# vanilladucky/sde_sampler_lrds

Hardware: AMD Instinct MI355X
Metric: particle-steps/sec (batch*n_steps/wall) + log-Z abs-err vs ref (higher is better)
Workload: dtype f32

## Files before the change

sde_sampler_lrds_amd/csrc/prep_kernels.hip:

```cpp
#include "sim_device.hpp"
#include "prep_kernels.hpp"

__global__ void __launch_bounds__(256) k_weight_scales(PackArgs a) {
  __shared__ float red[256];
  float* sc = a.out + sd_off_scales(a.NT);
  {
    const int l = blockIdx.x;
    const float* W = l == 0 ? a.w_in : (l == 1 ? a.w_h1 : (l == 2 ? a.w_h2 : a.w_out));
    const int n = (l == 0 || l == 3) ? SD_H * a.d : SD_H * SD_H;
    float m = 0.0f;
    for (int i = threadIdx.x; i < n; i += 256) {
      const float v = __builtin_fabsf(W[i]);
      m = (v <= 3.0e38f) ? fmaxf(m, v) : m;
    }
    red[threadIdx.x] = m;
    __syncthreads();
    for (int s = 128; s > 0; s >>= 1) {
      if (threadIdx.x < s) red[threadIdx.x] = fmaxf(red[threadIdx.x], red[threadIdx.x + s]);
      __syncthreads();
    }
    if (threadIdx.x == 0) {
      const float mx = red[0];
      int e = 0;
      if (mx > 0.0f && (mx < 9.765625e-4f || mx >= 16384.0f)) {
// ... 58 lines not shown
      a.out[sd_off_bias(NT) + b] = v;
    }
  }
}

__device__ inline float gelu_exact(float v) { return (v * 0.5f) * (1.0f + erff(v * 0.70710678118654752440f)); }

__global__ void __launch_bounds__(64) k_time_embed(TimeEmbedArgs a) {
  __shared__ float e[128];
  __shared__ float hbuf[2][64];
  const int k = blockIdx.x, j = threadIdx.x;
  const float t = a.t_direct ? a.t_value : a.coef[static_cast<size_t>(k) * SDENG_NCOEF + a.col];
  const float arg = (a.te.coeff[j] * t) + a.te.phase[j];
  e[j] = sinf(arg);
  e[64 + j] = cosf(arg);
  __syncthreads();
  const float* in = e;
  int n_in = 128, cur = 0;
  for (int l = 0; l < a.te.n_hidden; ++l) {
    const float* W = a.te.w[l] + static_cast<size_t>(j) * n_in;
    float acc = 0.0f;
    for (int i = 0; i < n_in; ++i) acc = __builtin_fmaf(W[i], in[i], acc);
    acc += a.te.b[l][j];
    hbuf[cur][j] = gelu_exact(acc);
    __syncthreads();
    in = hbuf[cur];
    n_in = 64;
    cur ^= 1;
  }
  if (j < a.te.dim_out) {
    const float* W = a.te.w_out + static_cast<size_t>(j) * 64;
    float acc = 0.0f;
    for (int i = 0; i < 64; ++i) acc = __builtin_fmaf(W[i], in[i], acc);
    acc += a.te.b_out[j];
    if (a.clip > 0.0f) acc = clampf(acc, a.clip);
    a.out[static_cast<size_t>(k) * a.te.dim_out + j] = acc;
  }
}

__global__ void __launch_bounds__(128) k_same_var(const float* vars, int K, int d, float* same_var) {
  int differ = 0;
  for (int i = threadIdx.x; i < K * d; i += 128) differ |= vars[i] != vars[i % d];
  differ = __syncthreads_or(differ);
  if (threadIdx.x == 0) same_var[0] = differ ? 0.0f : 1.0f;
}

__global__ void __launch_bounds__(128) k_ref_tables(RefTabArgs a) {
  __shared__ float red[128];
  const int k = blockIdx.x / a.K, c = blockIdx.x % a.K;
  const float S = a.coef[static_cast<size_t>(k) * SDENG_NCOEF + 9];
  const float VA = a.coef[static_cast<size_t>(k) * SDENG_NCOEF + 10];
  const float S2 = a.coef[static_cast<size_t>(k) * SDENG_NCOEF + 11];
  const bool centred = a.centred && a.K == SD_KREG && a.same_var[0] != 0.0f;
  float* tm = a.tab + (static_cast<size_t>(k) * a.K + c) * 2 * a.dpad;
  float* tv = tm + a.dpad;
  float ls = 0.0f, quad = 0.0f;
  for (int f = threadIdx.x; f < a.dpad; f += 128) {
    float mean = 0.0f, iv = 0.0f, cen = 0.0f;
    if (f < a.d) {
      mean = S * a.means[static_cast<size_t>(c) * a.d + f];
      const float var = VA + S2 * a.vars[static_cast<size_t>(c) * a.d + f];
      iv = 1.0f / var;
      ls += logf(var);
      if (centred) {
        float sum = 0.0f;
        for (int j = 0; j < SD_KREG; ++j) sum += a.means[static_cast<size_t>(j) * a.d + f];
        cen = S * (sum * (1.0f / SD_KREG));
      }
    }
    if (centred) {
      const float dm = mean - cen;
      quad = __builtin_fmaf(dm * dm, iv, quad);
      tm[f] = dm * iv;
      tv[f] = c == 0 ? iv : (c == 1 ? cen : 0.0f);
    } else {
      tm[f] = mean;
      tv[f] = iv;
    }
  }
  red[threadIdx.x] = ls;
  __syncthreads();
  for (int s = 64; s > 0; s >>= 1) {
    if (threadIdx.x < s) red[threadIdx.x] += red[threadIdx.x + s];
    __syncthreads();
  }
  const float ls_sum = red[0];
  __syncthreads();
  red[threadIdx.x] = quad;
  __syncthreads();
  for (int s = 64; s > 0; s >>= 1) {
    if (threadIdx.x < s) red[threadIdx.x] += red[threadIdx.x + s];
    __syncthreads();
  }
  if (threadIdx.x == 0) {
    float wsum = 0.0f;
    for (int i = 0; i < a.K; ++i) wsum += a.weights ? a.weights[i] : 1.0f;
    const float w = (a.weights ? a.weights[c] : 1.0f) / wsum;
    float* cs = a.consts + (static_cast<size_t>(k) * a.K + c) * 2;
    cs[0] = 0.5f * ls_sum;
    cs[1] = centred ? logf(w) - 0.5f * red[0] : logf(w);
  }
}

__global__ void __launch_bounds__(256) k_ref_full_tables(RefFullArgs a) {
  __shared__ float invd[128];
  __shared__ float red[256];
  const int k = blockIdx.x / a.K, c = blockIdx.x % a.K;
  const float S = a.coef ? a.coef[static_cast<size_t>(k) * SDENG_NCOEF + 9] : 1.0f;
  const float VA = a.coef ? a.coef[static_cast<size_t>(k) * SDENG_NCOEF + 10] : 0.0f;
  const float S2 = a.coef ? a.coef[static_cast<size_t>(k) * SDENG_NCOEF + 11] : 1.0f;
  const int KB = sd_kb(a.NT);
  const int img_floats = a.NT * KB * 512;
  float ls = 0.0f;
  for (int j = threadIdx.x; j < 128; j += 256) {
    float iv = 0.0f;
    if (j < a.d) {
      const float var = VA + S2 * a.eigvals[static_cast<size_t>(c) * a.d + j];
      iv = 1.0f / var;
      ls += logf(var);
    }
    invd[j] = iv;
  }
  red[threadIdx.x] = ls;
  __syncthreads();
  for (int s = 128; s > 0; s >>= 1) {
    if (threadIdx.x < s) red[threadIdx.x] += red[threadIdx.x + s];
    __syncthreads();
// ... 799 lines not shown
```

sde_sampler_lrds_amd/csrc/prep_kernels.hpp:

```cpp
#pragma once
#include "sim_common.hpp"
#include "../../include/sdeng.h"

#define SD_LOGZ_MAX_BLOCKS 1024

struct PackArgs {
  int NT, d;
  const float *w_in, *b_in, *w_h1, *b_h1, *w_h2, *b_h2, *w_out, *b_out;
  float* out;
  int transpose;
  const float* scales;
};

struct TimeEmbedArgs {
  sdeng_time_embed te;
  const float* coef;
  int col;
  int t_direct;
  float t_value;
  float clip;
  float* out;
};

struct RefTabArgs {
  int K, d, dpad;
  const float* coef;
  const float *means, *vars, *weights;
  float* tab;
  float* consts;
  float* same_var;
  int centred;
};

struct RefFullArgs {
  int K, d, dpad, NT;
  const float* coef;
  const float *means, *eigvals, *eigvecs, *weights;
  float* images;
  float* means_out;
  float* consts;
};

struct RefMMArgs {
  int K, d, dpad, NT, kt;
  const float* coef;
  const float *means, *vars, *weights;
  float* images;
  float* centre;
  float* consts;
  float* same_var;
};

struct DistTabArgs {
  int K, d, dpad;
  const float *loc, *scale, *weights;
  float* tab;
  float* consts;
};

struct DistEvalArgs {
  DistDev ds;
  int B, d, dpad;
  const float* x;
  float* logp_out;
  float* score_out;
};

struct MovesArgs {
  DistEvalArgs prior, target;
  int B, d, K, keep_from, ula;
  float target_acc;
  const float* t;
  float *x, *lp, *grad, *step;
  const float *z, *u;
  unsigned seed_lo, seed_hi;
  long long chain0;
  float* samples;
  float* acc_sum;
  float* acc_last;
};
int sd_launch_moves(const MovesArgs& a, hipStream_t s);

struct TerminalArgs {
  DistDev ref, target;
// ... 18 lines not shown
```

sde_sampler_lrds_amd/csrc/sdeng_api.hip:

```cpp
#include <hip/hip_runtime.h>

#include <algorithm>
#include <cmath>
#include <cstdarg>
#include <cstdio>
#include <cstring>
#include <cstdlib>

#include "../../include/sdeng.h"
#include "prep_kernels.hpp"
#include "sim_kernel.hpp"
#include "cmcd_kernel.hpp"
#include "grad_kernel.hpp"
#include "cmcd_adjoint_kernel.hpp"
#include "metric_kernels.hpp"

int sd_launch_logreg_images(const float* X, const float* y, int n, int dw, int NT, float* image, float* y_pad, hipStream_t s);
int sd_launch_pack_square(const float* P, const float* loc, int d, int NT, float* out, float* loc_pad, hipStream_t s);

static thread_local char g_err[512] = "";
static int fail(int code, const char* fmt, ...) {
  va_list ap;
  va_start(ap, fmt);
  vsnprintf(g_err, sizeof(g_err), fmt, ap);
// ... 500 lines not shown
  SD_TRY(launch_timed(d, p.k, &c, s));
  if (eubo) return terminal(d, dpad, prior, prior, true, false, d->x_out, d->rnd_out, s);
  return terminal(d, dpad, target, target, false, true, d->x_out, d->rnd_out, s);
}

static int run_euler(const SimPlan& p, const sdeng_desc* d, float* ws, SimArgs& a, hipStream_t s) {
  SD_TRY(build_dist(d->target, d->d, 16 * p.DT, ws + p.L.target, a.target, s));
  a.clip_score = d->net.clip_score;
  return launch_timed(d, p.k, &a, s);
}

static int prepare_ref(const SimPlan& p, const sdeng_desc* d, float* ws, SimArgs& a, hipStream_t s) {
  const Layout& L = p.L;
  const int DT = p.DT, dpad = 16 * DT, K = ref_components(d), rf = p.rf;
  if (rf == RF_NONE) return 0;
  a.ref_k = K;
  a.ref_tab = ws + L.ref_tab; a.ref_consts = ws + L.ref_consts;
  a.ref_c1 = half_d_log_2pi(d->d);
  if (rf == RF_GMM_FULL) {
    if (d->N > 0) {
      RefFullArgs r;
      r.K = K; r.d = d->d; r.dpad = dpad; r.NT = DT; r.coef = p.in_slot ? nullptr : d->coef;
      r.means = d->ref.means_init; r.eigvals = d->ref.vars_init; r.eigvecs = d->ref.eigvecs; r.weights = d->ref.weights;
      r.images = ws + L.ref_tab; r.means_out = ws + L.ref_mean; r.consts = ws + L.ref_consts;
      SD_HIP(sd_launch_ref_full_tables(r, d->N, s));
    }
    a.ref_mean = ws + L.ref_mean;
    const int piece = (DT > 4 ? DT / 2 : DT) * sd_kb(DT) * 512;
    a.ref_share = (piece / 256 + SD_WAVES - 1) / SD_WAVES;
    return 0;
  }
  if (rf == RF_GMM_MM) {
    const int kt = (K + 15) / 16;
    if (d->N > 0) {
      RefMMArgs r;
      r.K = K; r.d = d->d; r.dpad = dpad; r.NT = DT; r.kt = kt; r.coef = d->coef;
      r.means = d->ref.means_init; r.vars = d->ref.vars_init; r.weights = d->ref.weights;
      r.images = ws + L.ref_tab; r.centre = ws + L.ref_mean; r.consts = ws + L.ref_consts;
      r.same_var = ws + L.ref_consts + static_cast<size_t>(d->N) * 64;
      SD_HIP(sd_launch_ref_mm_tables(r, d->N, s));
    }
    a.ref_kc = kt;
    a.ref_mean = ws + L.ref_mean;
    a.ref_share = (mm_piece(K, DT) / 256 + SD_WAVES - 1) / SD_WAVES;
    return 0;
  }
  if (d->N > 0) {
    RefTabArgs r;
    r.K = K; r.d = d->d; r.dpad = dpad; r.coef = d->coef;
    r.means = d->ref.means_init; r.vars = d->ref.vars_init; r.weights = rf != RF_GAUSS ? d->ref.weights : nullptr;
    r.tab = ws + L.ref_tab; r.consts = ws + L.ref_consts;
    r.same_var = ws + L.ref_consts + static_cast<size_t>(d->N) * K * 2;
    r.centred = (rf == RF_GMM && p.k.fam != SD_FAM_SPLIT) ? 1 : 0;
    SD_HIP(sd_launch_ref_tables(r, d->N, s));
  }
  a.ref_same_var = ws + L.ref_consts + static_cast<size_t>(d->N) * K * 2;
  if (rf == RF_GMM_BIG) {
    static const bool allow = [] { const char* e = getenv("SDENG_REF_SHARE"); return !(e && e[0] == '0'); }();
    const int cap = std::min(share_room(DT), sd_share_buf_floats(SD_SHARE_MAX)) / 256 * 256;
    const int kc_max = cap / (2 * dpad);
    if (allow && kc_max >= 1) {
      const int nch = (K + kc_max - 1) / kc_max;
      const int kc = (K + nch - 1) / nch;
      const int chunks = (kc * 2 * dpad + 255) / 256;
      a.ref_share = (chunks + SD_WAVES - 1) / SD_WAVES;
      a.ref_kc = kc;
    }
  }
  return 0;
}

static int run_sim(const SimPlan& p, const sdeng_desc* d, float* ws, SimArgs& a, hipStream_t s) {
  const Layout& L = p.L;
  const int DT = p.DT, dpad = 16 * DT;
  SD_TRY(prepare_net(d, L, ws, DT, a, s, d->N, false, 0.0f));
  SD_TRY(prepare_ref(p, d, ws, a, s));
  DistDev target, ref_dist, prior;
  SD_TRY(build_dist(d->target, d->d, dpad, ws + L.target, target, s));
  SD_TRY(build_dist(d->ref_dist, d->d, dpad, ws + L.ref_dist, ref_dist, s));
  SD_TRY(build_dist(d->prior, d->d, dpad, ws + L.prior, prior, s));
  a.target = target;
  a.prior = prior;
  const bool eubo = d->form == SDENG_FORM_EUBO;
  const bool tr = d->flags & SDENG_FLAG_TERM_REF, tt = d->flags & SDENG_FLAG_TERM_TARGET;
  if ((d->flags & SDENG_FLAG_INIT_LOGP) && !eubo) {
    SD_TRY(dist_eval(prior, d->B, d->d, dpad, d->x_in, ws + L.rnd_init, nullptr, s));
    a.rnd_init = ws + L.rnd_init;
  }
  if (eubo && (tr || tt)) {
    SD_HIP(hipMemsetAsync(ws + L.rnd_init, 0, sizeof(float) * d->B, s));
    SD_TRY(terminal(d, dpad, ref_dist, target, tr, tt, d->x_in, ws + L.rnd_init, s));
    a.rnd_init = ws + L.rnd_init;
  }
  if (p.sc == SC_LOGREG) {
    float* unused;
    SD_TRY(prepare_logreg(d, L, ws, DT, a, s, &unused));
  }
  SD_TRY(launch_timed(d, p.k, &a, s));
  if (!eubo && (tr || tt)) SD_TRY(terminal(d, dpad, ref_dist, target, tr, tt, d->x_out, d->rnd_out, s));
  if (eubo && (d->flags & SDENG_FLAG_INIT_LOGP)) SD_TRY(terminal(d, dpad, prior, prior, true, false, d->x_out, d->rnd_out, s));
  return 0;
}

extern "C" int sdeng_simulate(const sdeng_desc* desc, void* stream) {
  hipStream_t s = static_cast<hipStream_t>(stream);
  SimPlan p;
// ... 145 lines not shown
}
static int check_adjoint(const sdeng_desc* d, bool ext_score) {
  if (!d) return fail(SDENG_E_INVALID, "null descriptor");
  SD_TRY(check_abi(d));
  if (d->d < 1 || d->d > 128 || d->N < 1 || d->B < 1 || !d->coef) return fail(SDENG_E_INVALID, "bad sizes (1 <= d <= 128, N, B >= 1) or null coef");
  if (d->form != SDENG_FORM_LIN && d->form != SDENG_FORM_EM) return fail(SDENG_E_UNSUPPORTED, "kl_adjoint: forward forms LIN / EM (form %d)", d->form);
  if (d->net.ctrl_kind != SDENG_CTRL_CLIPPED &&
      !(score_like(d->net.ctrl_kind) && (ext_score || d->target.kind == SDENG_DIST_GMM_DIAG || d->target.kind == SDENG_DIST_PHI4)))
    return fail(SDENG_E_UNSUPPORTED, "kl_adjoint: ClippedCtrl, or Score / Lerp / CancelDrift control on a diagonal mixture / phi^4 target (ctrl_kind %d, "
                                     "target kind %d)", d->net.ctrl_kind, d->target.kind);
  SD_TRY(check_lerp_prior(d));
  if (d->target.kind == SDENG_DIST_CHECKERBOARD || d->prior.kind == SDENG_DIST_CHECKERBOARD)
    return fail(SDENG_E_UNSUPPORTED, "kl_adjoint: no adjoint for a checkerboard target (KL training takes the per-step path)");
  if (d->ref.kind != SDENG_REF_NONE && d->ref.kind != SDENG_REF_GAUSS_DIAG && d->ref.kind != SDENG_REF_GMM_DIAG)
    return fail(SDENG_E_UNSUPPORTED, "kl_adjoint: no reference, or a diagonal Gaussian / mixture reference (ref.kind %d)", d->ref.kind);
  if (d->ref.kind != SDENG_REF_NONE && ((d->ref.kind == SDENG_REF_GMM_DIAG && d->ref.k < 1) || !d->ref.means_init || !d->ref.vars_init))
    return fail(SDENG_E_INVALID, "reference: null means/vars or k < 1");
  if (static_cast<long long>(d->N) * d->B * d->d >= (1ll << 31)) return fail(SDENG_E_UNSUPPORTED, "N * B * d >= 2^31");
  return check_net(d->net);
}
extern "C" size_t sdeng_kl_adjoint_workspace_bytes(const sdeng_desc* d) {
  if (!d || d->d < 1 || d->d > 128 || d->N < 1) return 0;
  return adjoint_layout(d, tiles_exact(d->d)).total * sizeof(float);
}
extern "C" int sdeng_kl_adjoint(const sdeng_desc* d, const sdeng_adjoint* adj, void* stream) {
  hipStream_t s = static_cast<hipStream_t>(stream);
  SD_TRY(check_adjoint(d, adj && adj->score));
  if (!adj || !adj->xs || !adj->w || !adj->lam_in || !adj->a0 || !adj->a1 || !adj->a2 || !adj->d0 || !adj->d1 || !adj->d2 || !adj->dout)
    return fail(SDENG_E_INVALID, "kl_adjoint: null states / weights / lambda_N / per-row outputs");
  const bool ito = d->flags & SDENG_FLAG_ITO;
  if (ito && !adj->noise) return fail(SDENG_E_INVALID, "kl_adjoint: FLAG_ITO needs the normals of the trajectory");
  const bool score = d->net.ctrl_kind != SDENG_CTRL_CLIPPED;
  if (score && !adj->dst) return fail(SDENG_E_INVALID, "kl_adjoint: a score control needs the dst output");
  if (score && !adj->score) SD_TRY(check_dist(d->target, d->d));
  const int has_score = !score ? ADJ_NONE : adj->score ? ADJ_EXT : (d->target.kind == SDENG_DIST_PHI4 ? ADJ_PHI4 : ADJ_GMM);
  const int DT = tiles_exact(d->d), dpad = 16 * DT;
  KernelKey k;
  SD_TRY(select_kernel(k, SD_FAM_ADJ, DT, has_score));
  const AdjLayout A = adjoint_layout(d, DT);
  const size_t need = A.total * sizeof(float);
  if (!d->workspace || d->workspace_bytes < need) return fail(SDENG_E_WORKSPACE, "workspace %zu bytes, need %zu", d->workspace_bytes, need);
  float* ws = static_cast<float*>(d->workspace);
  AdjArgs a;
  memset(&a, 0, sizeof(a));
  SD_TRY(pack_net(d, DT, ws, ws + A.v.wt, s));
  SD_TRY(embed_times(d, d->N, false, 0.0f, ws + A.v.temb, ws + A.stheta, &a.stheta, s));
  if (d->ref.kind != SDENG_REF_NONE) {
    const int K = ref_components(d);
    RefTabArgs r;
    r.K = K; r.d = d->d; r.dpad = dpad; r.coef = d->coef;
    r.means = d->ref.means_init; r.vars = d->ref.vars_init; r.weights = d->ref.kind == SDENG_REF_GMM_DIAG ? d->ref.weights : nullptr;
    r.tab = ws + A.tab; r.consts = ws + A.consts;
    r.same_var = ws + A.consts + static_cast<size_t>(d->N) * K * 2;
    r.centred = 0;
    SD_HIP(sd_launch_ref_tables(r, d->N, s));
    a.ref_tab = ws + A.tab; a.ref_consts = ws + A.consts; a.ref_k = K;
    a.ref_c1 = half_d_log_2pi(d->d);
  }
  a.has_score = has_score;
  if (score) {
    a.score_ext = adj->score;
    if (!adj->score) SD_TRY(build_dist(d->target, d->d, dpad, ws + A.target, a.target, s));
    a.scale_score = d->net.scale_score; a.clip_score = d->net.clip_score;
    a.ctrl_kind = d->net.ctrl_kind;
    a.prior_loc = d->prior.p0; a.prior_scale = d->net.ctrl_kind == SDENG_CTRL_LERP ? d->prior.p1 : 1.0f;
    a.score_detached = adj->detach_score ? 1 : 0;
    a.dst = adj->dst;
  }
  VjpArgs& v = a.v;
  v.M = d->N * d->B; v.B = d->B; v.d = d->d; v.N = d->N;
  v.x = adj->xs; v.cot = nullptr; v.wpack = ws; v.wpack_t = ws + A.v.wt; v.temb = ws + A.v.temb;
  v.clip_model = d->net.clip_model;
  v.a0 = adj->a0; v.a1 = adj->a1; v.a2 = adj->a2; v.d0 = adj->d0; v.d1 = adj->d1; v.d2 = adj->d2; v.dout = adj->dout;
  v.trash = ws + A.v.trash;
  a.coef = d->coef; a.noise = ito ? adj->noise : nullptr; a.w = adj->w; a.lam_in = adj->lam_in; a.lam_out = adj->lam_out;
  a.lin = d->form == SDENG_FORM_LIN ? 1 : 0;
  a.ntiles_b = (d->B + 15) / 16;
  SD_HIP(k.fn(&a, s));
  return 0;
}

struct CmcdAdjLayout {
  VjpLayout v;
  size_t stheta, target, prior, total;
};
static CmcdAdjLayout cmcd_adjoint_layout(const sdeng_desc* d, int DT) {
  CmcdAdjLayout A;
  A.v = vjp_layout(DT, d->N + 1);
  size_t o = A.v.total;
  A.stheta = o; o += align64(static_cast<size_t>(d->N) + 1);
  A.target = o; o += dist_floats(d->target, 16 * DT);
  A.prior = o; o += dist_floats(d->prior, 16 * DT);
  A.total = o;
  return A;
}
static int check_cmcd_adjoint(const sdeng_desc* d, bool ext_score) {
  if (!d) return fail(SDENG_E_INVALID, "null descriptor");
  SD_TRY(check_abi(d));
  if (d->d > 128) return fail(SDENG_E_UNSUPPORTED, "cmcd_kl_adjoint: d <= 128 (got %d)", d->d);
  if (d->d < 1 || d->N < 1 || d->B < 1 || !d->coef) return fail(SDENG_E_INVALID, "bad sizes (1 <= d, N, B >= 1) or null coef");
  if (d->net.ctrl_kind != SDENG_CTRL_CLIPPED && d->net.ctrl_kind != SDENG_CTRL_SCORE)
    return fail(SDENG_E_UNSUPPORTED, "cmcd_kl_adjoint: ClippedCtrl or ScoreCtrl (ctrl_kind %d)", d->net.ctrl_kind);
  if (d->prior.kind == SDENG_DIST_GAUSS_FULL)
    return fail(SDENG_E_UNSUPPORTED, "cmcd_kl_adjoint: no adjoint for a full-covariance prior (KL training takes the per-step path)");
  if (d->prior.kind != SDENG_DIST_ISO_GAUSS && d->prior.kind != SDENG_DIST_GAUSS_DIAG)
    return fail(SDENG_E_UNSUPPORTED, "cmcd_kl_adjoint: prior must be ISO_GAUSS or GAUSS_DIAG (kind %d)", d->prior.kind);
  switch (d->target.kind) {
// ... 204 lines not shown
```

sde_sampler_lrds_amd/csrc/sim_device.hpp:

```cpp
#pragma once
#include "sim_common.hpp"
#include "../../include/sdeng.h"

#define SD_INLINE __device__ __forceinline__

SD_INLINE float group_sum(float v) {
  v += __shfl_xor(v, 16, 64);
  v += __shfl_xor(v, 32, 64);
  return v;
}
SD_INLINE float exp_nonpos(float v) { return __builtin_amdgcn_exp2f(v * 1.4426950408889634f); }
SD_INLINE float rcp_fast(float v) { return __builtin_amdgcn_rcpf(v); }

SD_INLINE float clampf(float v, float m) {
  v = (v < -m) ? -m : v;
  v = (v > m) ? m : v;
  return v;
}

SD_INLINE void clamp_tile_rare(f32x4& v, float m) {
  bool out_of_range = false;
#pragma unroll
  for (int r = 0; r < 4; ++r) out_of_range |= !(__builtin_fabsf(v[r]) <= m);
  if (__builtin_amdgcn_ballot_w64(out_of_range) != 0) {
#pragma unroll
    for (int r = 0; r < 4; ++r) v[r] = clampf(v[r], m);
  }
}

SD_INLINE int feat(int t, int r, int g) { return 16 * t + 4 * g + r; }
SD_INLINE bool feat_lt(int t, int r, int g4, int d) { return g4 < d - (16 * t + r); }
template <int NT>
SD_INLINE bool feat_live(int t, int r, int g4, int d) { return (t < NT - 1) ? true : feat_lt(t, r, g4, d); }

SD_INLINE f32x4 load_tile4(const float* base, int t, int g) { return *reinterpret_cast<const f32x4*>(base + 16 * t + 4 * g); }

typedef _Float16 f16x8 __attribute__((ext_vector_type(8)));
#define SD_LO_SCALE 2048.0f
#define SD_LO_INV 4.8828125e-04f

typedef float f32x2 __attribute__((ext_vector_type(2)));
typedef _Float16 f16x2 __attribute__((ext_vector_type(2)));
SD_INLINE float opaque_one() {
  float one = 1.0f;
  asm("" : "+s"(one));
  return one;
}
SD_INLINE void split_pair(float a, float b, uint32_t& hi, uint32_t& lo) {
  const float one = opaque_one();
  const f16x2 h = __builtin_convertvector(f32x2{a, b}, f16x2);
  float d0 = __builtin_fmaf(a, one, -static_cast<float>(h[0]));
  float d1 = __builtin_fmaf(b, one, -static_cast<float>(h[1]));
  d0 *= SD_LO_SCALE;
  d1 *= SD_LO_SCALE;
  const f16x2 l = __builtin_convertvector(f32x2{d0, d1}, f16x2);
  hi = __builtin_bit_cast(uint32_t, h);
  lo = __builtin_bit_cast(uint32_t, l);
}
typedef uint32_t u32x4 __attribute__((ext_vector_type(4)));
SD_INLINE void split8(const f32x4& t0, const f32x4& t1, f16x8& hi, f16x8& lo) {
  uint32_t h0, h1, h2, h3, l0, l1, l2, l3;
  split_pair(t0[0], t0[1], h0, l0);
  split_pair(t0[2], t0[3], h1, l1);
  split_pair(t1[0], t1[1], h2, l2);
  split_pair(t1[2], t1[3], h3, l3);
  hi = __builtin_bit_cast(f16x8, u32x4{h0, h1, h2, h3});
  lo = __builtin_bit_cast(f16x8, u32x4{l0, l1, l2, l3});
}

SD_INLINE void split8_half(const f32x4& t0, f16x8& hi, f16x8& lo) {
  uint32_t h0, h1, l0, l1;
  split_pair(t0[0], t0[1], h0, l0);
  split_pair(t0[2], t0[3], h1, l1);
  hi = __builtin_bit_cast(f16x8, u32x4{h0, h1, 0u, 0u});
  lo = __builtin_bit_cast(f16x8, u32x4{l0, l1, 0u, 0u});
}

// ... 501 lines not shown
    if (k < K) {
      lp[k] = gmm_logit<NT>(x, tab, consts, cstride, k, c1, g);
      mx = fmaxf(mx, lp[k]);
    }
  }
  float den = 0.0f;
#pragma unroll
  for (int k = 0; k < SD_KREG; ++k) {
    p[k] = (k < K) ? exp_nonpos(lp[k] - mx) : 0.0f;
    den += p[k];
  }
  const float inv = rcp_fast(den);
#pragma unroll
  for (int k = 0; k < SD_KREG; ++k) p[k] *= inv;
}

template <int NT, int KC = 0>
SD_INLINE f32x4 gmm_score_tile(const f32x4 (&x)[NT], const float* __restrict__ tab, int K, int g, const float (&p)[SD_KREG], int t) {
  constexpr int dpad = 16 * NT;
  if constexpr (KC == SD_KREG) K = SD_KREG;
  f32x4 acc = {0.0f, 0.0f, 0.0f, 0.0f};
#pragma unroll
  for (int k = 0; k < SD_KREG; ++k) {
    if (k < K) {
      const float* mp = tab + static_cast<size_t>(k) * 2 * dpad;
      const f32x4 m = load_tile4(mp, t, g);
      const f32x4 iv = load_tile4(mp + dpad, t, g);
#pragma unroll
      for (int r = 0; r < 4; ++r) acc[r] = __builtin_fmaf(p[k], (m[r] - x[t][r]) * iv[r], acc[r]);
    }
  }
  return acc;
}

template <int NT, int KC = 0>
SD_INLINE f32x4 gmm_score_tile_shared_var(const f32x4 (&x)[NT], const float* __restrict__ tab, int K, int g, const float (&p)[SD_KREG], int t) {
  constexpr int dpad = 16 * NT;
  if constexpr (KC == SD_KREG) K = SD_KREG;
  f32x4 acc = {0.0f, 0.0f, 0.0f, 0.0f};
#pragma unroll
  for (int k = 0; k < SD_KREG; ++k) {
    if (k < K) {
      const f32x4 m = load_tile4(tab + static_cast<size_t>(k) * 2 * dpad, t, g);
#pragma unroll
      for (int r = 0; r < 4; ++r) acc[r] = __builtin_fmaf(p[k], m[r], acc[r]);
    }
  }
  const f32x4 iv = load_tile4(tab + dpad, t, g);
#pragma unroll
  for (int r = 0; r < 4; ++r) acc[r] = (acc[r] - x[t][r]) * iv[r];
  return acc;
}

template <int NT>
SD_INLINE void gmm_resp_centred(const f32x4 (&x)[NT], const float* __restrict__ tab, const float* __restrict__ consts, int g,
                                float (&p)[SD_KREG]) {
  constexpr int dpad = 16 * NT;
  float lp[SD_KREG];
#pragma unroll
  for (int k = 0; k < SD_KREG; ++k) lp[k] = 0.0f;
#pragma unroll
  for (int t = 0; t < NT; ++t) {
    const f32x4 y = x[t] - load_tile4(tab + 3 * dpad, t, g);
#pragma unroll
    for (int k = 0; k < SD_KREG; ++k) {
      const f32x4 ak = load_tile4(tab + static_cast<size_t>(k) * 2 * dpad, t, g);
#pragma unroll
      for (int r = 0; r < 4; ++r) lp[k] = __builtin_fmaf(y[r], ak[r], lp[k]);
    }
  }
  float mx = -INFINITY;
#pragma unroll
  for (int k = 0; k < SD_KREG; ++k) {
    lp[k] = consts[2 * k + 1] + group_sum(lp[k]);
    mx = fmaxf(mx, lp[k]);
  }
  float den = 0.0f;
#pragma unroll
  for (int k = 0; k < SD_KREG; ++k) {
    p[k] = exp_nonpos(lp[k] - mx);
    den += p[k];
  }
  const float inv = rcp_fast(den);
#pragma unroll
  for (int k = 0; k < SD_KREG; ++k) p[k] *= inv;
}
template <int NT>
SD_INLINE f32x4 gmm_score_tile_centred(const f32x4 (&x)[NT], const float* __restrict__ tab, int g, const float (&p)[SD_KREG], int t) {
  constexpr int dpad = 16 * NT;
  f32x4 acc = {0.0f, 0.0f, 0.0f, 0.0f};
#pragma unroll
  for (int k = 0; k < SD_KREG; ++k) {
    const f32x4 ak = load_tile4(tab + static_cast<size_t>(k) * 2 * dpad, t, g);
#pragma unroll
    for (int r = 0; r < 4; ++r) acc[r] = __builtin_fmaf(p[k], ak[r], acc[r]);
  }
  const f32x4 iv = load_tile4(tab + dpad, t, g), c = load_tile4(tab + 3 * dpad, t, g);
#pragma unroll
  for (int r = 0; r < 4; ++r) acc[r] = __builtin_fmaf(c[r] - x[t][r], iv[r], acc[r]);
  return acc;
}

template <int NT>
SD_INLINE f32x4 gauss_score_tile(const f32x4 (&x)[NT], const float* __restrict__ tab, int g, int t) {
  constexpr int dpad = 16 * NT;
  const f32x4 m = load_tile4(tab, t, g);
  const f32x4 iv = load_tile4(tab + dpad, t, g);
  f32x4 out;
#pragma unroll
  for (int r = 0; r < 4; ++r) out[r] = -((x[t][r] - m[r]) * iv[r]);
  return out;
}

SD_INLINE f32x4 rings_score(const f32x4& x, const DistDev& ds, int g) {
  const float n = __builtin_sqrtf(x[0] * x[0] + x[1] * x[1]) + 1e-7f;
  const float var = ds.p0 * ds.p0;
  float wsum = 0.0f;
  for (int k = 0; k < ds.k; ++k) wsum += ds.aux1[k];
  const float cn = 0.5f * 1.8378770664093453f + 0.5f * logf(var);
  float lp[8], mx = -INFINITY;
#pragma unroll
  for (int k = 0; k < 8; ++k) {
    lp[k] = -INFINITY;
    if (k < ds.k) {
      const float dl = n - ds.aux0[k];
      lp[k] = logf(ds.aux1[k] / wsum) + ((-0.5f * ((dl * dl) / var)) - cn);
      mx = fmaxf(mx, lp[k]);
    }
  }
  float den = 0.0f, acc = 0.0f;
#pragma unroll
  for (int k = 0; k < 8; ++k) {
    if (k < ds.k) {
      const float e = expf(lp[k] - mx);
      den += e;
      acc += e * ((n - ds.aux0[k]) / var);
    }
  }
  const float sr = -(acc / den);
  const float f = (sr / n) - (1.0f / (n * n));
  return g == 0 ? f32x4{x[0] * f, x[1] * f, 0.0f, 0.0f} : f32x4{0.0f, 0.0f, 0.0f, 0.0f};
}

template <int NT>
SD_INLINE void phi4_edges(const f32x4 (&x)[NT], int t, int g, int lane, float& l_edge, float& r_edge) {
  const int up = (lane + 48) & 63, dn = (lane + 16) & 63;
  const float l_same = __shfl(x[t][3], up, 64);
  const float r_same = __shfl(x[t][0], dn, 64);
  float l_prev = 0.0f, r_next = 0.0f;
  if (t > 0) l_prev = __shfl(x[t > 0 ? t - 1 : 0][3], up, 64);
  if (t < NT - 1) r_next = __shfl(x[t < NT - 1 ? t + 1 : t][0], dn, 64);
  l_edge = (g == 0) ? l_prev : l_same;
// ... 138 lines not shown
```

sde_sampler_lrds_amd/csrc/sim_kernel.hpp:

```cpp
#pragma once
#include <type_traits>

#include "sim_device.hpp"

enum { RF_NONE = 0, RF_GAUSS = 1, RF_GMM = 2, RF_GMM_BIG = 3, RF_GMM_FULL = 4, RF_GMM_MM = 5 };
enum { SC_NONE = 0, SC_GMM = 1, SC_PHI4 = 2, SC_LOGREG = 3, SC_REFSLOT = 4 };

template <int KIND, bool CLIP>
SD_INLINE float ctrl_score_term(const SimArgs& a, float sv, float xv, float st, float score_gain, float lerp_w, bool in_range,
                                float inv_prior_var) {
  constexpr bool lerp = KIND == SDENG_CTRL_LERP;
  if constexpr (lerp) {
    const float ps = (a.prior.p0 - xv) * inv_prior_var;
    const float df = sv - ps;
    sv = (lerp_w < 0.5f) ? ps + lerp_w * df : sv - df * (1.0f - lerp_w);
  }
  if constexpr (CLIP) sv = clampf(sv, a.clip_score);
  float v = a.scale_score * sv;
  v = v * st;
  if constexpr (lerp) v = in_range ? score_gain * v : 0.0f;
  if constexpr (KIND == SDENG_CTRL_CANCEL_DRIFT) v = in_range ? lerp_w * xv + score_gain * v : 0.0f;
  return v;
}
template <int KIND, bool CLIP>
// ... 78 lines not shown
    if constexpr (SC == SC_LOGREG) {
      const int ni = a.lr.in_lds ? sd_lr_floats(NT, a.lr.n_rows) / 4 : 0;
      for (int i = tid; i < ni; i += THREADS) dst[n4 + i] = reinterpret_cast<const f32x4*>(a.lr.image)[i];
    }
  }
  __syncthreads();
#ifdef SD_STAGGER
  if constexpr (REF != RF_GMM_BIG && REF != RF_GMM_FULL && REF != RF_GMM_MM)
    if (wave >= W / 2)
      for (int i = 0; i < SD_STAGGER; ++i) __builtin_amdgcn_s_sleep(127);
#endif
#ifdef SD_DBG_PRIO_HI47
  if (wave >= 4) __builtin_amdgcn_s_setprio(3);
#endif
#ifdef SD_DBG_ONLY47
  if (wave < 4) return;
#endif
#ifdef SD_DBG_ONLY03
  if (wave >= 4) return;
#endif
  static_assert(SC != SC_LOGREG || (REF == RF_NONE && NT <= 4), "in-loop logistic-regression score: no reference, d <= 64");
  static_assert(SC != SC_REFSLOT || (REF == RF_GMM_FULL && FORM != SDENG_FORM_EUBO), "full-covariance target score: lives in the reference slot, forward forms");
  constexpr bool has_ref = REF != RF_NONE && SC != SC_REFSLOT;
  const float* bias = a.wpack + sd_off_bias(NT);
  const NetScale ns = load_net_scale(bias, NT);
#ifdef SD_NO_RANGE_GUARD
  const bool scaled_net = false;
#else
  const bool scaled_net = ns.any_hidden();
#endif
  const float inv_out_plain = ns.inv_out;
#ifdef SD_DBG_NODMA
  constexpr bool ref_lds = false;
#else
  constexpr bool ref_lds = (REF == RF_GAUSS || REF == RF_GMM);
#endif
  float* my_tab = lds + sd_lds_weight_floats(NT) + wave * SD_REFTAB_FLOATS;
  const int tab_floats = a.ref_k * 2 * dpad;
  const int share = (REF == RF_GMM_BIG || REF == RF_GMM_FULL || REF == RF_GMM_MM) ? __builtin_amdgcn_readfirstlane(a.ref_share) : 0;
  float* sh_tab = lds + sd_lds_weight_floats(NT);
  const int sh_floats = sd_share_buf_floats(share);
  constexpr int FULL_PP = NT > 4 ? 2 : 1, FULL_TO = NT / FULL_PP, FULL_PIECE = FULL_TO * ((NT + 1) / 2) * 512;
  static_assert(REF != RF_GMM_FULL || NT % FULL_PP == 0, "pieces hold whole output tiles");
  const int p = lane & 15, g = lane >> 4;
  constexpr bool lin = FORM == SDENG_FORM_LIN;
  constexpr bool eubo = FORM == SDENG_FORM_EUBO;
  static_assert(!eubo || (SC == SC_NONE) != (REF == RF_NONE), "EUBO kernels: reference-SDE losses with a ClippedCtrl, or DIS (no reference)");
  const bool full_d = a.d == dpad;
  float* trash = a.trash + tid * 4;
  bool same_var = false;
  if constexpr (REF == RF_GMM) same_var = a.N > 0 && a.ref_same_var[0] != 0.0f;
  const bool kfull = REF == RF_GMM && a.ref_k == SD_KREG;
  const bool kfast = kfull && same_var;

  for (int tile = blockIdx.x + gridDim.x * wave; (share ? tile - static_cast<int>(gridDim.x) * wave : tile) < a.ntiles;
       tile += gridDim.x * W) {
    const uint32_t row = static_cast<uint32_t>(tile) * 16u + p;
    const bool live = row < static_cast<uint32_t>(a.B);
    const uint32_t pidx = static_cast<uint32_t>(a.particle0 + row);
    f32x4 x[NT];
    load_rows<NT>(a.x_in, row, a.d, live, g, x);
    float rnd = 0.0f;
    if (a.rnd_init) rnd = (live ? a.rnd_init[row] : 0.0f);
    if constexpr (PAR) {
      if (a.xs_out) store_rows<NT>(a.xs_out, trash, row, a.d, live, g, x);
    }
    if constexpr (ref_lds) {
      if (a.N > 0) dma_table_to_lds(a.ref_tab, my_tab, tab_floats, lane);
    }
    if constexpr (REF == RF_GMM_BIG) {
      if (share) {
        __syncthreads();
        if (a.N > 0) dma_table_shared(a.ref_tab, sh_tab, min(a.ref_kc, a.ref_k) * 2 * dpad, share, wave, lane);
      }
    }
    if constexpr (REF == RF_GMM_MM) {
      __syncthreads();
      if (a.N > 0) dma_table_shared(a.ref_tab, sh_tab, a.ref_kc * ((NT + 1) / 2) * 512, share, wave, lane);
    }
    if constexpr (REF == RF_GMM_FULL) {
      __syncthreads();
      if (a.N > 0) dma_table_shared(a.ref_tab, sh_tab, FULL_PIECE, share, wave, lane);
    }

    for (int k = 0; k < a.N; ++k) {
      const float* cf = a.coef + static_cast<size_t>(k) * SDENG_NCOEF;
      const float c1 = cf[1], c2 = cf[2], c3 = cf[3], c4 = cf[4], c5 = cf[5], c6 = cf[6];
      const float score_gain = cf[7], lerp_w = cf[8];
      const float e1 = __builtin_fmaf(c4, c1, 1.0f), e2 = c4 * c2, e3 = c4 * c3, e4 = c2 * c5;
      int d_dyn = a.d;
      asm volatile("" : "+s"(d_dyn));

      auto noise_tile = [&](int t) -> f32x4 {
        if (PAR && a.noise_in) return load_quad(a.noise_in + static_cast<size_t>(k) * a.B * a.d, row, d_dyn, live, t, g);
        f32x4 z = philox_normal4(pidx, static_cast<uint32_t>(k), static_cast<uint32_t>(4 * t + g), 0u, a.seed_lo, a.seed_hi);
        if constexpr (SC == SC_PHI4) {
          if (!full_d) {
#pragma unroll
            for (int r = 0; r < 4; ++r) z[r] = feat_live<NT>(t, r, 4 * g, d_dyn) ? z[r] : 0.0f;
          }
        }
        return z;
      };
      if constexpr (eubo) {
#pragma unroll
        for (int t = 0; t < NT; ++t) {
          const f32x4 z = noise_tile(t);
#pragma unroll
          for (int r = 0; r < 4; ++r) x[t][r] = x[t][r] * c1 + c3 * z[r];
        }
      }

      f32x4 hid[SD_HT];
      __builtin_amdgcn_s_setprio(2);
      constexpr bool has_twin = REF != RF_GMM_MM && REF != RF_GMM_FULL && SC != SC_LOGREG;
      if constexpr (has_twin) mlp_hidden<NT>(x, hid, lds, bias, a.temb + static_cast<size_t>(k) * SD_H, lane);
      else mlp_hidden_scaled<NT>(x, hid, lds, bias, a.temb + static_cast<size_t>(k) * SD_H, lane, ns);
      __builtin_amdgcn_s_setprio(1);
      HidSplit hs = split_hidden(hid);
      bool safe_net = false;
      float hid_rs = 1.0f;

      f32x4 ts[(SC != SC_NONE && SC != SC_REFSLOT) ? NT : 1];
      if constexpr (SC == SC_GMM) {
        if (NT == 1 && a.target.kind == SDENG_DIST_RINGS) ts[0] = rings_score(x[0], a.target, g);
        else gmm_score<NT>(x, a.target.tab, a.target.consts, 4, a.target.k, a.target.p0, g, ts);
      }
      if constexpr (SC == SC_PHI4) {
        int lane_p = lane;
        if constexpr (NT == 8) asm volatile("" : "+v"(lane_p));
        phi4_score<NT>(x, a.target, d_dyn, g, lane_p, ts);
      }
      if constexpr (SC == SC_LOGREG) {
        asm volatile("" ::: "memory");
        f16x8 xh[(NT + 1) / 2], xl[(NT + 1) / 2];
        split_tiles<NT>(x, xh, xl);
        if (a.lr.in_lds) logreg_score<NT>(x, xh, xl, a.lr, d_dyn, lds + sd_lds_weight_floats(NT), lane, ts);
        else logreg_score<NT>(x, xh, xl, a.lr, d_dyn, a.lr.image, lane, ts);
      }
      const float* rtab = ref_lds ? my_tab : a.ref_tab + static_cast<size_t>(k) * tab_floats;
      const float* rcs = a.ref_consts + static_cast<size_t>(k) * a.ref_k * 2;
      if constexpr (ref_lds) wait_dma();
      float resp[REF == RF_GMM ? SD_KREG : 1];
      f32x4 rs[(REF == RF_GMM_BIG || REF == RF_GMM_FULL || REF == RF_GMM_MM) ? NT : 1];
#ifdef SD_DBG_NOREF
      if constexpr (REF == RF_GMM) { resp[0] = 1.0f; resp[1] = resp[2] = resp[3] = 0.0f; }
#else
      if constexpr (REF == RF_GMM) {
        if (kfast) gmm_resp_centred<NT>(x, rtab, rcs, g, resp);
        else if (kfull) gmm_resp<NT, SD_KREG>(x, rtab, rcs, 2, SD_KREG, a.ref_c1, g, resp);
        else gmm_resp<NT>(x, rtab, rcs, 2, a.ref_k, a.ref_c1, g, resp);
      }
#endif
      if constexpr (REF == RF_GMM_BIG) {
        if (share) {
          const int kc = a.ref_kc, nch = (a.ref_k + kc - 1) / kc;
          float m_run, l_run;
          gmm_score_begin<NT>(rs, m_run, l_run);
          for (int c = 0; c < nch; ++c) {
            const int q = k * nch + c;
            wait_dma();
            __syncthreads();
            const int c2 = c + 1 < nch ? c + 1 : 0, k2 = c + 1 < nch ? k : k + 1;
            if (k2 < a.N)
              dma_table_shared(a.ref_tab + static_cast<size_t>(k2) * tab_floats + c2 * kc * 2 * dpad,
                               sh_tab + ((q + 1) & 1) * sh_floats, min(kc, a.ref_k - c2 * kc) * 2 * dpad, share, wave, lane);
            gmm_score_accum<NT>(x, sh_tab + (q & 1) * sh_floats, rcs + c * kc * 2, 2, min(kc, a.ref_k - c * kc), a.ref_c1, g, rs,
                                m_run, l_run);
          }
          gmm_score_end<NT>(rs, l_run);
        } else {
          gmm_score<NT>(x, rtab, rcs, 2, a.ref_k, a.ref_c1, g, rs);
        }
      }
      if constexpr (REF == RF_GMM_MM) {
        constexpr int KBX = (NT + 1) / 2, KTM = 4;
        const int kt = a.ref_kc, kbk = (kt + 1) / 2;
        const float* cs = a.ref_mean + static_cast<size_t>(k) * 2 * dpad;
        const float* bk = a.ref_consts + static_cast<size_t>(k) * (KTM * 16);
        const int logit_floats = kt * KBX * 512, mean_floats = NT * kbk * 512;
        const float* img = a.ref_tab + static_cast<size_t>(k) * (logit_floats + mean_floats);
        f16x8 ch[KBX], cl[KBX];
        {
          f32x4 xc[NT];
#pragma unroll
          for (int t = 0; t < NT; ++t) xc[t] = x[t] - load_tile4(cs, t, g);
          split_tiles<NT>(xc, ch, cl);
        }
        wait_dma();
        __syncthreads();
        dma_table_shared(img + logit_floats, sh_tab + sh_floats, mean_floats, share, wave, lane);
        f32x4 lt[KTM];
        {
          const f16x8* im = reinterpret_cast<const f16x8*>(sh_tab);
#pragma unroll
          for (int j = 0; j < KTM; ++j) {
            lt[j] = f32x4{-INFINITY, -INFINITY, -INFINITY, -INFINITY};
            if (j < kt) {
              f32x4 acc = load_tile4(bk, j, g), mx = {0.0f, 0.0f, 0.0f, 0.0f};
#pragma unroll
              for (int kb = 0; kb < KBX; ++kb) {
                const f16x8 ah = im[((j * KBX + kb) * 2 + 0) * 64 + lane], al = im[((j * KBX + kb) * 2 + 1) * 64 + lane];
// ... 111 lines not shown
      float st = 1.0f;
      if constexpr (SC != SC_NONE) st = a.stheta ? a.stheta[k] : 1.0f;

      float su2 = 0.0f, suz = 0.0f, sux = 0.0f;
      constexpr bool can_remove = SC != SC_NONE && has_ref && !eubo;
      auto ref_tile = [&](int t) __attribute__((always_inline)) -> f32x4 {
        f32x4 rq = {0.0f, 0.0f, 0.0f, 0.0f};
#ifdef SD_DBG_NOREF
        if constexpr (REF == RF_GMM) rq = f32x4{resp[0], resp[0], resp[0], resp[0]};
#else
        if constexpr (REF == RF_GMM) {
          if (kfast) rq = gmm_score_tile_centred<NT>(x, rtab, g, resp, t);
          else if (kfull) rq = gmm_score_tile<NT, SD_KREG>(x, rtab, SD_KREG, g, resp, t);
          else rq = same_var ? gmm_score_tile_shared_var<NT>(x, rtab, a.ref_k, g, resp, t) : gmm_score_tile<NT>(x, rtab, a.ref_k, g, resp, t);
        }
#endif
        if constexpr (REF == RF_GMM_BIG || REF == RF_GMM_FULL || REF == RF_GMM_MM) rq = rs[t];
        if constexpr (REF == RF_GAUSS) rq = gauss_score_tile<NT>(x, rtab, g, t);
        return rq;
      };
      auto out_group = [&](auto otc, int t0) __attribute__((always_inline)) {
        constexpr int OT = decltype(otc)::value;
        f32x4 u[OT];
        if constexpr (has_twin) {
          mlp_out_tiles<NT, OT>(hs, lds, bias, t0, lane, u);
          if (__builtin_expect(safe_net, 0)) out_tiles_unscale<OT>(u, bias, t0, lane, hid_rs, ns.inv_out);
          else if (__builtin_expect(inv_out_plain != 1.0f, 0)) {
            asm volatile("" ::: "memory");
#pragma unroll
            for (int o = 0; o < OT; ++o) u[o] = u[o] * inv_out_plain;
          }
        } else {
          mlp_out_tiles<NT, OT>(hs, lds, bias, t0, lane, u, ns.inv_out);
        }
#ifdef SD_NO_RANGE_GUARD
        constexpr bool range_guard = false;
#else
        constexpr bool range_guard = has_twin;
#endif
        if (has_twin && t0 == 0) {
          const bool bad = range_guard && !(__builtin_fabsf(u[0][0]) <= 3.0e38f);
          const bool trip = scaled_net | (__builtin_amdgcn_ballot_w64(bad) != 0);
          if (__builtin_expect(trip, 0)) {
            asm volatile("" ::: "memory");
            safe_net = true;
            mlp_hidden_safe<NT>(x, hid, lds, bias, a.temb + static_cast<size_t>(k) * SD_H, lane, ns);
            hid_rs = split_hidden_safe(hid, hs);
            mlp_out_tiles<NT, OT>(hs, lds, bias, t0, lane, u);
            out_tiles_unscale<OT>(u, bias, t0, lane, hid_rs, ns.inv_out);
            asm volatile("" ::: "memory");
          }
        }
        if (a.clip_model > 0.0f) {
          bool out_of_range = false;
#pragma unroll
          for (int o = 0; o < OT; ++o)
#pragma unroll
            for (int r = 0; r < 4; ++r) out_of_range |= !(__builtin_fabsf(u[o][r]) <= a.clip_model);
          if (__builtin_amdgcn_ballot_w64(out_of_range) != 0) {
#pragma unroll
            for (int o = 0; o < OT; ++o)
#pragma unroll
              for (int r = 0; r < 4; ++r) u[o][r] = clampf(u[o][r], a.clip_model);
          }
        }
#pragma unroll
        for (int o = 0; o < OT; ++o) {
          const int t = t0 + o;
          if constexpr (SC == SC_REFSLOT) add_ctrl_score_tile(a, u[o], rs[t], x[t], st, score_gain, lerp_w, t, 4 * g, d_dyn);
          else if constexpr (SC != SC_NONE) add_ctrl_score_tile(a, u[o], ts[t], x[t], st, score_gain, lerp_w, t, 4 * g, d_dyn);
          f32x4 rq = {0.0f, 0.0f, 0.0f, 0.0f};
          if constexpr (can_remove) {
            rq = ref_tile(t);
            if (a.flags & SDENG_FLAG_REMOVE_REF) u[o] = u[o] - rq;
          }
          if constexpr (PAR == 2) perturb_ctrl_tile<NT, REF != RF_GMM_FULL>(a, cf, u[o], x[t], pidx, k, t, g, d_dyn);
#pragma unroll
          for (int r = 0; r < 4; ++r) {
            float uv = u[o][r];
            if constexpr (eubo) uv = uv * c2;
            u[o][r] = uv;
            if constexpr (!eubo) su2 = __builtin_fmaf(uv, uv, su2);
          }
          const f32x4 z = noise_tile(t);
          if constexpr (!can_remove && has_ref) rq = ref_tile(t);
#pragma unroll
          for (int r = 0; r < 4; ++r) {
            const float xv = x[t][r], uv = u[o][r];
            if constexpr (eubo) {
              su2 += uv * (rq[r] + 0.5f * uv);
              sux = __builtin_fmaf(uv, xv, sux);
              suz = __builtin_fmaf(uv, z[r], suz);
            } else if constexpr (lin) {
              float sc = uv;
              if constexpr (has_ref) sc = rq[r] + uv;
              x[t][r] = __builtin_fmaf(c3, z[r], __builtin_fmaf(c2, sc, c1 * xv));
              suz = __builtin_fmaf(uv, z[r], suz);
            } else {
              float acc = e1 * xv;
              if constexpr (has_ref) acc = __builtin_fmaf(e3, rq[r], acc);
              x[t][r] = __builtin_fmaf(e4, z[r], __builtin_fmaf(e2, uv, acc));
              suz = __builtin_fmaf(uv, z[r], suz);
            }
          }
        }
      };
#pragma unroll
      for (int t0 = 0; t0 < NT; t0 += 2) {
        if (t0 + 1 < NT) out_group(std::integral_constant<int, 2>{}, t0);
        else out_group(std::integral_constant<int, 1>{}, t0);
      }
      __builtin_amdgcn_s_setprio(0);
      if constexpr (ref_lds) {
        __builtin_amdgcn_sched_barrier(0);
        if (k + 1 < a.N) dma_table_to_lds(a.ref_tab + static_cast<size_t>(k + 1) * tab_floats, my_tab, tab_floats, lane);
      }
      su2 = group_sum(su2);
      if constexpr (eubo) {
        rnd -= su2 * c4;
        if (c6 != 0.0f) rnd += group_sum(sux) * c6;
        rnd -= group_sum(suz) * c5;
      } else {
        rnd += lin ? c4 * su2 : (0.5f * su2) * c4;
        rnd += c6;
        if (a.flags & SDENG_FLAG_ITO) {
          suz = group_sum(suz);
          rnd += c5 * suz;
        }
      }
      if constexpr (PAR) {
        if (a.xs_out) store_rows<NT>(a.xs_out + static_cast<size_t>(k + 1) * a.B * a.d, trash, row, d_dyn, live, g, x);
      }
    }

    store_rows<NT>(a.x_out, trash, row, a.d, live, g, x);
    if (live && g == 0) a.rnd_out[row] = rnd;
  }
// ... 77 lines not shown
```

Measured before the change: 3.628 billion.

## Fold GMM reference score into precomputed affine update tables for LIN/EM forms

Precomputes per-step alpha/beta coefficients into spare rows of the centred GMM reference table, so the state update becomes x*A + B + sum_k p_k*a_k + gamma*u + delta*z. The responsibilities are pre-scaled by the step coefficient, which avoids recomputing the reference score tile and its separate combination. It also replaces the per-element out-of-range boolean OR in the clip checks with a max-abs reduction. The folded tables are computed in double then rounded, and the fold changes f32 rounding order. The max-based check treats NaN differently than the old test.

```diff
diff --git a/sde_sampler_lrds_amd/csrc/prep_kernels.hip b/sde_sampler_lrds_amd/csrc/prep_kernels.hip
--- a/sde_sampler_lrds_amd/csrc/prep_kernels.hip
+++ b/sde_sampler_lrds_amd/csrc/prep_kernels.hip
@@ -134,6 +134,13 @@
   const float VA = a.coef[static_cast<size_t>(k) * SDENG_NCOEF + 10];
   const float S2 = a.coef[static_cast<size_t>(k) * SDENG_NCOEF + 11];
   const bool centred = a.centred && a.K == SD_KREG && a.same_var[0] != 0.0f;
+  float alpha = 0.0f, beta = 0.0f;
+  {
+    const float* cf = a.coef + static_cast<size_t>(k) * SDENG_NCOEF;
+    if (a.form == SDENG_FORM_LIN) { alpha = cf[1]; beta = cf[2]; }
+    if (a.form == SDENG_FORM_EM) { alpha = __builtin_fmaf(cf[4], cf[1], 1.0f); beta = cf[4] * cf[3]; }
+  }
+  const bool folded = a.form == SDENG_FORM_LIN || a.form == SDENG_FORM_EM;
   float* tm = a.tab + (static_cast<size_t>(k) * a.K + c) * 2 * a.dpad;
   float* tv = tm + a.dpad;
   float ls = 0.0f, quad = 0.0f;
@@ -154,7 +161,12 @@
       const float dm = mean - cen;
       quad = __builtin_fmaf(dm * dm, iv, quad);
       tm[f] = dm * iv;
-      tv[f] = c == 0 ? iv : (c == 1 ? cen : 0.0f);
+      float row = c == 0 ? iv : cen;
+      if (c >= 2) {
+        const double bi = static_cast<double>(beta) * static_cast<double>(iv);
+        row = (folded && f < a.d) ? static_cast<float>(c == 2 ? static_cast<double>(alpha) - bi : bi * static_cast<double>(cen)) : 0.0f;
+      }
+      tv[f] = row;
     } else {
       tm[f] = mean;
       tv[f] = iv;
diff --git a/sde_sampler_lrds_amd/csrc/prep_kernels.hpp b/sde_sampler_lrds_amd/csrc/prep_kernels.hpp
--- a/sde_sampler_lrds_amd/csrc/prep_kernels.hpp
+++ b/sde_sampler_lrds_amd/csrc/prep_kernels.hpp
@@ -30,6 +30,7 @@
   float* consts;
   float* same_var;
   int centred;
+  int form;
 };
 
 struct RefFullArgs {
diff --git a/sde_sampler_lrds_amd/csrc/sdeng_api.hip b/sde_sampler_lrds_amd/csrc/sdeng_api.hip
--- a/sde_sampler_lrds_amd/csrc/sdeng_api.hip
+++ b/sde_sampler_lrds_amd/csrc/sdeng_api.hip
@@ -576,6 +576,7 @@
     r.tab = ws + L.ref_tab; r.consts = ws + L.ref_consts;
     r.same_var = ws + L.ref_consts + static_cast<size_t>(d->N) * K * 2;
     r.centred = (rf == RF_GMM && p.k.fam != SD_FAM_SPLIT) ? 1 : 0;
+    r.form = d->form;
     SD_HIP(sd_launch_ref_tables(r, d->N, s));
   }
   a.ref_same_var = ws + L.ref_consts + static_cast<size_t>(d->N) * K * 2;
@@ -827,7 +828,7 @@
     r.means = d->ref.means_init; r.vars = d->ref.vars_init; r.weights = d->ref.kind == SDENG_REF_GMM_DIAG ? d->ref.weights : nullptr;
     r.tab = ws + A.tab; r.consts = ws + A.consts;
     r.same_var = ws + A.consts + static_cast<size_t>(d->N) * K * 2;
-    r.centred = 0;
+    r.centred = 0; r.form = d->form;
     SD_HIP(sd_launch_ref_tables(r, d->N, s));
     a.ref_tab = ws + A.tab; a.ref_consts = ws + A.consts; a.ref_k = K;
     a.ref_c1 = half_d_log_2pi(d->d);
diff --git a/sde_sampler_lrds_amd/csrc/sim_device.hpp b/sde_sampler_lrds_amd/csrc/sim_device.hpp
--- a/sde_sampler_lrds_amd/csrc/sim_device.hpp
+++ b/sde_sampler_lrds_amd/csrc/sim_device.hpp
@@ -18,11 +18,29 @@
   return v;
 }
 
+template <int T>
+SD_INLINE bool any_beyond(const f32x4 (&v)[T], float m) {
+#ifdef SD_NO_CLIPMAX
+  bool out_of_range = false;
+#pragma unroll
+  for (int t = 0; t < T; ++t)
+#pragma unroll
+    for (int r = 0; r < 4; ++r) out_of_range |= !(__builtin_fabsf(v[t][r]) <= m);
+  return out_of_range;
+#else
+  float acc = 0.0f;
+#pragma unroll
+  for (int t = 0; t < T; ++t) {
+    acc = __builtin_fmaxf(__builtin_fmaxf(__builtin_fabsf(v[t][0]), __builtin_fabsf(v[t][1])), acc);
+    acc = __builtin_fmaxf(__builtin_fmaxf(__builtin_fabsf(v[t][2]), __builtin_fabsf(v[t][3])), acc);
+  }
+  return acc > m;
+#endif
+}
+
 SD_INLINE void clamp_tile_rare(f32x4& v, float m) {
-  bool out_of_range = false;
-#pragma unroll
-  for (int r = 0; r < 4; ++r) out_of_range |= !(__builtin_fabsf(v[r]) <= m);
-  if (__builtin_amdgcn_ballot_w64(out_of_range) != 0) {
+  const f32x4 one[1] = {v};
+  if (__builtin_amdgcn_ballot_w64(any_beyond<1>(one, m)) != 0) {
 #pragma unroll
     for (int r = 0; r < 4; ++r) v[r] = clampf(v[r], m);
   }
@@ -630,9 +648,9 @@
   return acc;
 }
 
-template <int NT>
+template <int NT, bool SCALED = false>
 SD_INLINE void gmm_resp_centred(const f32x4 (&x)[NT], const float* __restrict__ tab, const float* __restrict__ consts, int g,
-                                float (&p)[SD_KREG]) {
+                                float (&p)[SD_KREG], float scale = 1.0f) {
   constexpr int dpad = 16 * NT;
   float lp[SD_KREG];
 #pragma unroll
@@ -659,7 +677,8 @@
     p[k] = exp_nonpos(lp[k] - mx);
     den += p[k];
   }
-  const float inv = rcp_fast(den);
+  float inv = rcp_fast(den);
+  if constexpr (SCALED) inv = inv * scale;
 #pragma unroll
   for (int k = 0; k < SD_KREG; ++k) p[k] *= inv;
 }
@@ -676,6 +695,25 @@
   const f32x4 iv = load_tile4(tab + dpad, t, g), c = load_tile4(tab + 3 * dpad, t, g);
 #pragma unroll
   for (int r = 0; r < 4; ++r) acc[r] = __builtin_fmaf(c[r] - x[t][r], iv[r], acc[r]);
+  return acc;
+}
+
+template <int NT>
+SD_INLINE f32x4 gmm_update_tile_folded(const f32x4 (&x)[NT], const float* __restrict__ tab, int g, const float (&pb)[SD_KREG], int t,
+                                       const f32x4& u, const f32x4& z, float gamma, float delta) {
+  constexpr int dpad = 16 * NT;
+  const f32x4 A = load_tile4(tab + 5 * dpad, t, g), Bc = load_tile4(tab + 7 * dpad, t, g);
+  f32x4 acc;
+#pragma unroll
+  for (int r = 0; r < 4; ++r) acc[r] = __builtin_fmaf(A[r], x[t][r], Bc[r]);
+#pragma unroll
+  for (int k = 0; k < SD_KREG; ++k) {
+    const f32x4 ak = load_tile4(tab + static_cast<size_t>(k) * 2 * dpad, t, g);
+#pragma unroll
+    for (int r = 0; r < 4; ++r) acc[r] = __builtin_fmaf(pb[k], ak[r], acc[r]);
+  }
+#pragma unroll
+  for (int r = 0; r < 4; ++r) acc[r] = __builtin_fmaf(delta, z[r], __builtin_fmaf(gamma, u[r], acc[r]));
   return acc;
 }
 
diff --git a/sde_sampler_lrds_amd/csrc/sim_kernel.hpp b/sde_sampler_lrds_amd/csrc/sim_kernel.hpp
--- a/sde_sampler_lrds_amd/csrc/sim_kernel.hpp
+++ b/sde_sampler_lrds_amd/csrc/sim_kernel.hpp
@@ -154,6 +154,11 @@
   if constexpr (REF == RF_GMM) same_var = a.N > 0 && a.ref_same_var[0] != 0.0f;
   const bool kfull = REF == RF_GMM && a.ref_k == SD_KREG;
   const bool kfast = kfull && same_var;
+#if defined(SD_NO_FOLD) || defined(SD_DBG_NOREF)
+  constexpr bool can_fold = false;
+#else
+  constexpr bool can_fold = REF == RF_GMM && SC == SC_NONE && FORM != SDENG_FORM_EUBO;
+#endif
 
   for (int tile = blockIdx.x + gridDim.x * wave; (share ? tile - static_cast<int>(gridDim.x) * wave : tile) < a.ntiles;
        tile += gridDim.x * W) {
@@ -249,7 +254,7 @@
       if constexpr (REF == RF_GMM) { resp[0] = 1.0f; resp[1] = resp[2] = resp[3] = 0.0f; }
 #else
       if constexpr (REF == RF_GMM) {
-        if (kfast) gmm_resp_centred<NT>(x, rtab, rcs, g, resp);
+        if (kfast) gmm_resp_centred<NT, can_fold>(x, rtab, rcs, g, resp, lin ? c2 : e3);
         else if (kfull) gmm_resp<NT, SD_KREG>(x, rtab, rcs, 2, SD_KREG, a.ref_c1, g, resp);
         else gmm_resp<NT>(x, rtab, rcs, 2, a.ref_k, a.ref_c1, g, resp);
       }
@@ -467,12 +472,7 @@
           }
         }
         if (a.clip_model > 0.0f) {
-          bool out_of_range = false;
-#pragma unroll
-          for (int o = 0; o < OT; ++o)
-#pragma unroll
-            for (int r = 0; r < 4; ++r) out_of_range |= !(__builtin_fabsf(u[o][r]) <= a.clip_model);
-          if (__builtin_amdgcn_ballot_w64(out_of_range) != 0) {
+          if (__builtin_amdgcn_ballot_w64(any_beyond<OT>(u, a.clip_model)) != 0) {
 #pragma unroll
             for (int o = 0; o < OT; ++o)
 #pragma unroll
@@ -498,6 +498,14 @@
             if constexpr (!eubo) su2 = __builtin_fmaf(uv, uv, su2);
           }
           const f32x4 z = noise_tile(t);
+          if constexpr (can_fold) {
+            if (kfast) {
+              x[t] = gmm_update_tile_folded<NT>(x, rtab, g, resp, t, u[o], z, lin ? c2 : e2, lin ? c3 : e4);
+#pragma unroll
+              for (int r = 0; r < 4; ++r) suz = __builtin_fmaf(u[o][r], z[r], suz);
+              continue;
+            }
+          }
           if constexpr (!can_remove && has_ref) rq = ref_tile(t);
 #pragma unroll
           for (int r = 0; r < 4; ++r) {
```

After: 3.577 billion. 0.986x the previous value.
